# nv-tlabs/ChronoEdit

Hardware: AMD Instinct MI355X
Metric: denoising-steps/sec (higher is better)
Workload: dtype bf16

## Files before the change

### chronoedit_amd/csrc/ce_attn.hip

```cpp
#include <cstdlib>

#include "ce_common.h"

namespace {

constexpr int HD = 128;
constexpr int QW = 32;
constexpr int KVB = 64;
constexpr int K_TILE_BYTES = KVB * HD * 2;
constexpr int VT_TILE_BYTES = HD * KVB * 2;
constexpr int BUF_BYTES = K_TILE_BYTES + VT_TILE_BYTES;
constexpr int OST_ROW = HD * 2 + 16;
constexpr int smem_bytes(int nwave, bool two_seg) {
  const int stage = nwave * QW * OST_ROW;
  return two_seg ? 2 * BUF_BYTES + stage : (stage > 2 * BUF_BYTES ? stage : 2 * BUF_BYTES);
}
constexpr float NEG_BIG = -1.0e30f;

__device__ __forceinline__ int vt_swz(int dv) {
  return ((((dv >> 2) & 7) << 1) | (((dv >> 1) ^ (dv >> 5)) & 1)) ^ (((dv >> 6) & 1) << 1);
}

struct KVSeg {
  const bf16* k;
// ... 1377 lines not shown
#endif
  if (g_attn_nwave == 128 || g_attn_nwave == 129) {
    static bool done4_[CE_MAX_DEVICES] = {};
    bool& done4 = done4_[ce_device_slot()];
    if (!done4) {
      (void)hipFuncSetAttribute((const void*)attn_fwd_w4_kernel, hipFuncAttributeMaxDynamicSharedMemorySize, W4_SMEM);
      done4 = true;
    }
    const int grid4 = (g_attn_nwave == 129 && items > cus) ? (cus & ~7) : items;
    hipLaunchKernelGGL(attn_fwd_w4_kernel, dim3(grid4), dim3(256), W4_SMEM, stream, (const bf16*)Q, (bf16*)O, s0, Nq, H, ldq, ldo, nqb,
                       sl2, batch, blk);
    return (int)hipGetLastError();
  }
  const int grid_vt = items <= 2 * cus ? items : ((2 * cus) & ~7);
  hipLaunchKernelGGL((attn_fwd_sp_kernel<false, true>), dim3(grid_vt), dim3(512), sp_smem_bytes(false), stream, (const bf16*)Q, (bf16*)O,
                     s0, s1, Nq, H, ldq, ldo, nqb, sl2, batch, blk);
  return (int)hipGetLastError();
}

CE_API int ce_attention_vt_bf16(const void* Q, const void* K, const void* Vt, int len, int ldk, int ldvt, void* O, int Nq, int H,
                                    int head_dim, int ldq, int ldo, float softmax_scale, int batch, hipStream_t stream) {
  return attention_vt_launch(Q, K, Vt, len, ldk, ldvt, O, Nq, H, head_dim, ldq, ldo, softmax_scale, batch, 0, 0, 0, stream);
}

CE_API int ce_attention_vt_blocked_bf16(const void* Q, const void* K, const void* Vt, int len, int ldk, int ldvt, void* O, int Nq, int H,
                                            int head_dim, int ldq, int ldo, float softmax_scale, int batch, int blk_rows, int blk_stride,
                                            int vt_sample_cols, hipStream_t stream) {
  if (blk_rows <= 0) return CE_ERR_SHAPE;
  return attention_vt_launch(Q, K, Vt, len, ldk, ldvt, O, Nq, H, head_dim, ldq, ldo, softmax_scale, batch, blk_rows, blk_stride, vt_sample_cols,
                             stream);
}


static int attention_2seg_vt_launch(const void* Q, const void* K1, const void* V1t, int len1, int ldk1, int ldv1t, int vt_cols1,
                                    const void* K2, const void* V2t, int len2, int ldk2, int ldv2t, int vt_cols2, void* O, int Nq,
                                    int H, int head_dim, int ldq, int ldo, float softmax_scale, int batch, void* O8, void* S8, int ldo8,
                                    int q_rows, int k1_rows, int k2_rows, hipStream_t stream, const void* valid1 = nullptr,
                                    const void* w1 = nullptr) {
  if (!Q || !K1 || !V1t || !K2 || !V2t || (!O && !O8)) return CE_ERR_ARG;
  if ((valid1 != nullptr) != (w1 != nullptr) || (valid1 && O8)) return CE_ERR_ARG;
  if ((q_rows != 0 && q_rows < Nq) || (k1_rows != 0 && k1_rows < len1) || (k2_rows != 0 && k2_rows < len2)) return CE_ERR_SHAPE;
  if (k1_rows == 0) vt_cols1 = 0;
  if (k2_rows == 0) vt_cols2 = 0;
  if (head_dim != HD || Nq <= 0 || H <= 0 || len1 <= 0 || len2 <= 0 || batch <= 0 || batch > 65535) return CE_ERR_SHAPE;
  const int c1 = (len1 + KVB - 1) / KVB * KVB, c2 = (len2 + KVB - 1) / KVB * KVB;
  if ((k1_rows != 0 && vt_cols1 < len1) || (k2_rows != 0 && vt_cols2 < len2) || ldv1t < (batch - 1) * vt_cols1 + c1 || ldv2t < (batch - 1) * vt_cols2 + c2)
    return CE_ERR_SHAPE;
  if ((ldq & 7) || (ldo & 7) || (ldk1 & 7) || (ldk2 & 7) || (ldv1t & 7) || (ldv2t & 7) || (vt_cols1 & 1) || (vt_cols2 & 1)) return CE_ERR_ALIGN;
  KVSeg s0{(const bf16*)K1, (const bf16*)V1t, len1, ldk1, ldv1t};
  KVSeg s1{(const bf16*)K2, (const bf16*)V2t, len2, ldk2, ldv2t};
  const float sl2 = softmax_scale * 1.4426950408889634f;
  const int nqb = (Nq + 8 * QW - 1) / (8 * QW);
  static bool done_[CE_MAX_DEVICES] = {};
  bool& done = done_[ce_device_slot()];
  if (!done) {
    (void)hipFuncSetAttribute((const void*)attn_fwd_sp_kernel<true, true>, hipFuncAttributeMaxDynamicSharedMemorySize, sp_smem_bytes(true));
    (void)hipFuncSetAttribute((const void*)attn_fwd_sp_kernel<true, true, true>, hipFuncAttributeMaxDynamicSharedMemorySize, sp_smem_bytes(true));
    (void)hipFuncSetAttribute((const void*)attn_fwd_sp_kernel<true, true, false, true>, hipFuncAttributeMaxDynamicSharedMemorySize, sp_smem_bytes(true));
    done = true;
  }
  const BlkRows blk{0, vt_cols2, 0u, vt_cols1, (unsigned char*)O8, (unsigned char*)S8, ldo8, q_rows, k1_rows, k2_rows,
                    (const int*)valid1, (const float*)w1};
  const int cus = ce_device_cus();
  const int items = nqb * H * batch;
  const int grid = items <= 2 * cus ? items : ((2 * cus) & ~7);
  if (valid1)
    hipLaunchKernelGGL((attn_fwd_sp_kernel<true, true, false, true>), dim3(grid), dim3(512), sp_smem_bytes(true), stream, (const bf16*)Q,
                       (bf16*)O, s0, s1, Nq, H, ldq, ldo, nqb, sl2, batch, blk);
  else if (O8)
    hipLaunchKernelGGL((attn_fwd_sp_kernel<true, true, true>), dim3(grid), dim3(512), sp_smem_bytes(true), stream, (const bf16*)Q,
                       (bf16*)O, s0, s1, Nq, H, ldq, ldo, nqb, sl2, batch, blk);
  else
    hipLaunchKernelGGL((attn_fwd_sp_kernel<true, true>), dim3(grid), dim3(512), sp_smem_bytes(true), stream, (const bf16*)Q, (bf16*)O,
                       s0, s1, Nq, H, ldq, ldo, nqb, sl2, batch, blk);
  return (int)hipGetLastError();
}

CE_API int ce_attention_2seg_vt_bf16(const void* Q, const void* K1, const void* V1t, int len1, int ldk1, int ldv1t, int vt_cols1,
                                         const void* K2, const void* V2t, int len2, int ldk2, int ldv2t, int vt_cols2, void* O, int Nq,
                                         int H, int head_dim, int ldq, int ldo, float softmax_scale, int batch, hipStream_t stream) {
  if (!O) return CE_ERR_ARG;
  return attention_2seg_vt_launch(Q, K1, V1t, len1, ldk1, ldv1t, vt_cols1, K2, V2t, len2, ldk2, ldv2t, vt_cols2, O, Nq, H, head_dim, ldq, ldo,
                                  softmax_scale, batch, nullptr, nullptr, 0, Nq, len1, len2, stream);
}

CE_API int ce_attention_2seg_vt_strided_bf16(const void* Q, const void* K1, const void* V1t, int len1, int ldk1, int ldv1t, int vt_cols1,
                                                 const void* K2, const void* V2t, int len2, int ldk2, int ldv2t, int vt_cols2, void* O, int Nq,
                                                 int H, int head_dim, int ldq, int ldo, float softmax_scale, int batch, int q_rows, int k1_rows,
                                                 int k2_rows, hipStream_t stream) {
  if (!O) return CE_ERR_ARG;
  return attention_2seg_vt_launch(Q, K1, V1t, len1, ldk1, ldv1t, vt_cols1, K2, V2t, len2, ldk2, ldv2t, vt_cols2, O, Nq, H, head_dim, ldq, ldo,
                                  softmax_scale, batch, nullptr, nullptr, 0, q_rows, k1_rows, k2_rows, stream);
}

CE_API int ce_attention_2seg_vt_weighted_bf16(const void* Q, const void* K1, const void* V1t, int len1, int ldk1, int ldv1t, int vt_cols1,
                                                  const void* K2, const void* V2t, int len2, int ldk2, int ldv2t, int vt_cols2, void* O, int Nq,
                                                  int H, int head_dim, int ldq, int ldo, float softmax_scale, int batch, int q_rows, int k1_rows,
                                                  int k2_rows, const void* valid1, const void* w1, hipStream_t stream) {
  if (!O || !valid1 || !w1) return CE_ERR_ARG;
  return attention_2seg_vt_launch(Q, K1, V1t, len1, ldk1, ldv1t, vt_cols1, K2, V2t, len2, ldk2, ldv2t, vt_cols2, O, Nq, H, head_dim, ldq, ldo,
                                  softmax_scale, batch, nullptr, nullptr, 0, q_rows, k1_rows, k2_rows, stream, valid1, w1);
}

CE_API int ce_attention_2seg_vt_quant_bf16(const void* Q, const void* K1, const void* V1t, int len1, int ldk1, int ldv1t, int vt_cols1,
                                               const void* K2, const void* V2t, int len2, int ldk2, int ldv2t, int vt_cols2, void* o8,
                                               void* scale8, int Nq, int H, int head_dim, int ldq, int ldo8, float softmax_scale, int batch,
                                               hipStream_t stream) {
  if (!o8 || !scale8 || (ldo8 & 15) || ((H * head_dim) & 127)) return CE_ERR_ARG;
  return attention_2seg_vt_launch(Q, K1, V1t, len1, ldk1, ldv1t, vt_cols1, K2, V2t, len2, ldk2, ldv2t, vt_cols2, nullptr, Nq, H, head_dim, ldq,
                                  8, softmax_scale, batch, o8, scale8, ldo8, Nq, len1, len2, stream);
}
```

### chronoedit_amd/hiplib.py

```python
from __future__ import annotations

import ctypes
import os
import re
import subprocess
from typing import Dict, List

PKG_DIR = os.path.dirname(os.path.abspath(__file__))
ROOT = os.path.dirname(PKG_DIR)
CSRC = os.path.join(PKG_DIR, "csrc")
LIB_DIR = os.path.join(PKG_DIR, "lib")
LIB_PATH = os.path.join(LIB_DIR, "libchronoedit_hip.so")
DIAG_LIB_PATH = os.path.join(LIB_DIR, "libchronoedit_hip_diag.so")
OBJ_DIR = os.path.join(LIB_DIR, "obj")
HEADER = os.path.join(ROOT, "include", "chronoedit_hip.h")
DIAG_HEADER = os.path.join(ROOT, "include", "chronoedit_hip_diag.h")

DIAG_SOURCES = ["ce_gemm.hip", "ce_gemm256.hip", "ce_attn.hip", "ce_attn_fp8.hip", "ce_gemm_fp8.hip", "ce_gemm_fp8w4.hip"]
DIAG_ONLY_SOURCES = ["ce_attn16.hip"]
SOURCES = ["ce_rowops.hip", "ce_gemm.hip", "ce_gemm256.hip", "ce_gemm256w4.hip", "ce_gemm384.hip", "ce_attn.hip", "ce_attn16.hip", "ce_attn_fp8.hip", "ce_sched.hip", "ce_conv.hip", "ce_enc.hip", "ce_gemm_fp8.hip", "ce_gemm_fp8w4.hip", "ce_comm.hip", "ce_lora.hip", "ce_tea.hip", "ce_image.hip", "ce_region.hip", "ce_sparse.hip", "ce_region_auto.hip", "ce_focus.hip", "ce_autofocus.hip", "ce_preview.hip", "ce_lift.hip", "ce_sketch.hip", "ce_components.hip", "ce_clusters.hip", "ce_layers.hip"]

_c = ctypes
_P, _I, _F = _c.c_void_p, _c.c_int, _c.c_float

SIGNATURES: Dict[str, List] = {
    "ce_ln_affine_bf16": [_P, _P, _P, _P, _I, _I, _I, _I, _F, _I, _I, _P],
    "ce_rmsnorm_rope_bf16": [_P, _P, _P, _P, _P, _I, _I, _I, _I, _F, _I, _P],
    "ce_gemm_bf16": [_P, _P, _P, _P, _I, _P, _P, _I, _I, _I, _I, _I, _I, _I, _I, _I, _c.c_longlong, _I, _c.c_longlong, _P, _c.c_size_t, _P],
    "ce_gemm_bf16_res": [_P, _P, _P, _P, _I, _P, _P, _I, _I, _I, _I, _I, _I, _I, _I, _I, _I, _c.c_longlong, _I, _c.c_longlong, _P, _c.c_size_t, _P],
    "ce_rmsnorm_rope_mxfp8": [_P, _P, _P, _P, _P, _I, _I, _I, _I, _I, _F, _I, _F, _P],
    "ce_v_mxfp8_transpose": [_P, _I, _P, _P, _I, _I, _I, _I, _P],
    "ce_attention_mxfp8": [_P, _P, _P, _P, _P, _P, _P, _I, _I, _I, _I, _I, _I, _I, _I, _I, _P],
    "ce_attention_mxfp8_quant": [_P, _P, _P, _P, _P, _P, _P, _P, _I, _I, _I, _I, _I, _I, _I, _I, _I, _P],
    "ce_attention_mxfp8_add": [_P, _P, _P, _P, _P, _P, _P, _I, _P, _I, _P, _P, _I, _I, _I, _I, _I, _I, _I, _I, _I, _P],
    "ce_rope_scatter_bf16": [_P, _I, _P, _I, _I, _I, _I, _I, _P, _I, _P, _I, _P, _P, _I, _F, _I, _P],
    "ce_patchify_rows_bf16": [_P, _P, _I, _I, _I, _I, _I, _I, _I, _P],
    "ce_comm_load": [ctypes.c_char_p],
    "ce_comm_unique_id": [_P],
    "ce_comm_init": [ctypes.POINTER(ctypes.c_void_p), _P, _I, _I],
    "ce_comm_destroy": [_P],
    "ce_comm_all_to_all": [_P, _P, _P, ctypes.c_size_t, _P],
    "ce_comm_all_gather": [_P, _P, _P, ctypes.c_size_t, _P],
    "ce_ln_affine_fp8": [_P, _P, _P, _P, _P, _I, _I, _I, _I, _F, _I, _I, _P],
    "ce_quant_rows_fp8": [_P, _P, _P, _I, _I, _I, _I, _P],
    "ce_gemm_fp8": [_P, _P, _P, _P, _P, _P, _I, _P, _P, _I, _I, _I, _I, _I, _I, _I, _I, _P, _c.c_size_t, _P],
    "ce_quant_rows_mxfp8": [_P, _P, _P, _I, _I, _I, _I, _P],
    "ce_quant_rows_mxfp8_w": [_P, _P, _P, _I, _I, _I, _I, _P],
    "ce_ln_affine_mxfp8": [_P, _P, _P, _P, _P, _I, _I, _I, _I, _F, _I, _I, _P],
    "ce_gemm_mxfp8": [_P, _P, _P, _P, _P, _P, _I, _P, _P, _I, _I, _I, _I, _I, _I, _I, _I, _P, _c.c_size_t, _P],
    "ce_gemm_mxfp8_gelu_quant": [_P, _P, _P, _P, _P, _P, _P, _I, _I, _I, _I, _I, _I, _P, _c.c_size_t, _P],
    "ce_gemm_batched_bf16": [_P, _P, _P, _P, _I, _I, _I, _I, _I, _I, _I, _I, _I] + [ctypes.c_longlong] * 6 + [_P],
    "ce_im2col_patch2d_bf16": [_P, _P, _I, _I, _I, _I, _I, _I, _P],
    "ce_gather_rows_bf16": [_P, _P, _P, _I, _I, _I, _I, _I, _P],
    "ce_rmsnorm_bf16": [_P, _P, _P, _I, _I, _I, _I, _F, _P],
    "ce_softmax_t5_bf16": [_P, _P, _I, _I, _I, _I, _I, _I, _P, _P, _P, _P],
    "ce_attention_bf16": [_P, _P, _P, _I, _I, _I, _P, _P, _I, _I, _I, _P, _I, _I, _I, _I, _I, _F, _P],
    "ce_attention_batched_bf16": [_P, _P, _P, _I, _I, _I, _P, _P, _I, _I, _I, _P, _I, _I, _I, _I, _I, _F, _I, _P],
    "ce_attention_vt_bf16": [_P, _P, _P, _I, _I, _I, _P, _I, _I, _I, _I, _I, _F, _I, _P],
    "ce_attention_2seg_vt_bf16": [_P, _P, _P, _I, _I, _I, _I, _P, _P, _I, _I, _I, _I, _P, _I, _I, _I, _I, _I, _F, _I, _P],
    "ce_attention_2seg_vt_strided_bf16": [_P, _P, _P, _I, _I, _I, _I, _P, _P, _I, _I, _I, _I, _P, _I, _I, _I, _I, _I, _F, _I, _I, _I, _I, _P],
    "ce_attention_2seg_vt_weighted_bf16": [_P, _P, _P, _I, _I, _I, _I, _P, _P, _I, _I, _I, _I, _P, _I, _I, _I, _I, _I, _F, _I, _I, _I, _I, _P, _P, _P],
    "ce_attention_2seg_vt_quant_bf16": [_P, _P, _P, _I, _I, _I, _I, _P, _P, _I, _I, _I, _I, _P, _P, _I, _I, _I, _I, _I, _F, _I, _P],
    "ce_v_transpose_bf16": [_P, _I, _P, _I, _I, _I, _P],
    "ce_attention_vt_blocked_bf16": [_P, _P, _P, _I, _I, _I, _P, _I, _I, _I, _I, _I, _F, _I, _I, _I, _I, _P],
    "ce_v_transpose_blocked_bf16": [_P, _I, _P, _I, _I, _I, _I, _I, _I, _I, _P],
    "ce_timestep_sinusoid": [_P, _P, _I, _P],
    "ce_timestep_sinusoid_f32": [_P, _P, _I, _P],
    "ce_gemv": [_P, _I, _P, _P, _P, _I, _I, _I, _P],
    "ce_modulation": [_P, _P, _P, _I, _I, _I, _I, _I, _P],
    "ce_patchify_bf16": [_P, _P, _I, _I, _I, _I, _I, _P],
    "ce_unpatchify_bf16": [_P, _P, _I, _I, _I, _I, _I, _P],
    "ce_conv_igemm_bf16": [_P, _I, _P, _P, _P, _I, _P] + [_I] * 16 + [_P],
    "ce_conv3d_head_bf16": [_P, _I, _P, _P, _P, _I] + [_I] * 10 + [_P],
    "ce_gemm_bf16_tile_rows": [_I, _I, _I, _I, _c.c_longlong],
    "ce_zero_border_bf16": [_P, _I, _I, _I, _I, _I, _P],
    "ce_conv3d_gemm_bf16": [_P, _P, _I, _P, _P, _P, _I, _I, _I, _I, _I, _I, _I, _I, _P],
    "ce_conv3d_gemm_rms_silu_bf16": [_P, _P, _I, _P, _P, _P, _P, _I, _I, _I, _I, _I, _I, _I, _P, _I, _P],
    "ce_rms_silu_bf16": [_P, _P, _P, _c.c_longlong, _I, _I, _I, _I, _I, _I, _P],
    "ce_upsample2x_bf16": [_P, _P, _I, _I, _I, _I, _P],
    "ce_softmax_rows_f32_bf16": [_P, _P, _I, _I, _I, _I, _I, _F, _P],
    "ce_attention_1head_bf16": [_P, _P, _P, _P, _I, _I, _I, _I, _I, _I, _I, _F, _P, _c.c_longlong, _P],
    "ce_cfg_unipc_step": [_P, _P, _P, _P, _P, _P, _P, _P, _P, _c.c_longlong, _I, _P],
    "ce_cfg_unipc_step_delta": [_P, _P, _P, _P, _P, _P, _P, _P, _P, _c.c_longlong, _I, _I, _I, _P, _c.c_longlong, _P, _I, _P],
    "ce_lora_merge_bf16": [_P, _I, _P, _I, _I, _I, _I, _P, _P, _P, _P, _P],
    "ce_tea_rel_l1_bf16": [_P, _I, _I, _P, _P],
    "ce_tea_store_bf16": [_P, _P, _c.c_longlong, _P],
    "ce_tea_apply_bf16": [_P, _P, _c.c_longlong, _P],
    "ce_tea_store_dist_bf16": [_P, _P, _P, _P, _P, _c.c_longlong, _c.c_longlong, _P],
    "ce_image_resample_u8": [_P, _P, _I, _I, _I, _I, _P, _P, _I, _P],
    "ce_image_u8_lut_planar": [_P, _I, _I, _I, _I, _I, _I, _P, _P, _I, _P],
    "ce_video_to_u8": [_P, _P, _I, _I, _I, _I, _I, _P],
    "ce_region_weights_u8": [_P, _P, _I, _I, _P],
    "ce_region_blend_f32": [_P, _P, _P, _P, _P, _c.c_longlong, _c.c_longlong, _I, _P],
    "ce_region_composite": [_P, _I, _P, _P, _P, _I, _I, _I, _I, _P],
# ... 152 lines not shown
```

### chronoedit_amd/ops.py

```python
from __future__ import annotations

import ctypes
from typing import Optional

import torch

from . import hiplib

EPI_BIAS, EPI_BIAS_GELU, EPI_GATE_RES, EPI_BIAS_GELU_ERF = 0, 1, 2, 3
EPI_F32, EPI_MUL, EPI_BIAS_ROW, EPI_BIAS_T = 4, 5, 6, 7

_lib = None
_product = None

_KNOB_DEFAULTS = {"ce_set_gemm_variant": -1, "ce_set_attention_waves": 0, "ce_set_gemm_fp8_variant": 1,
                  "ce_set_attention_mxfp8_variant": 1, "ce_set_attention_mxfp8_persistent": 512}
_knobs = dict(_KNOB_DEFAULTS)


def lib():
    global _lib, _product
    if _lib is None:
        _lib = _product = hiplib.load()
        import os
# ... 389 lines not shown


def attention_2seg_vt_shared(q: torch.Tensor, k1: torch.Tensor, v1t: torch.Tensor, len1: int, k2: torch.Tensor, v2t: torch.Tensor, len2: int,
                             heads: int, out: torch.Tensor, batch: int, share_q: bool = False, share1: bool = False, share2: bool = False,
                             cols1: Optional[int] = None, cols2: Optional[int] = None, scale: Optional[float] = None):
    for n, t in (("q", q), ("k1", k1), ("v1t", v1t), ("k2", k2), ("v2t", v2t), ("out", out)):
        _dev(t, torch.bfloat16, n)
    Nq, Dq, ldq = _rows(q, "q")
    _, _, ldk1 = _rows(k1, "k1")
    _, _, ldk2 = _rows(k2, "k2")
    No, Do, ldo = _rows(out, "out")
    nq = Nq if share_q else Nq // batch
    assert Dq == heads * 128 and Do == Dq and v1t.shape[0] == Dq and v2t.shape[0] == Dq and v1t.stride(1) == 1 and v2t.stride(1) == 1
    assert No == batch * nq and (share_q or Nq == batch * nq), (No, Nq, batch)
    assert k1.shape[0] == (1 if share1 else batch) * len1 and k2.shape[0] == (1 if share2 else batch) * len2
    pad = lambda n: (n + 63) // 64 * 64
    if cols1 is None:
        cols1 = 0 if share1 else v1t.shape[1] // batch
    if cols2 is None:
        cols2 = 0 if share2 else v2t.shape[1] // batch
    assert v1t.shape[1] >= (0 if share1 else (batch - 1) * cols1) + pad(len1) and v2t.shape[1] >= (0 if share2 else (batch - 1) * cols2) + pad(len2)
    if scale is None:
        scale = 128 ** -0.5
    st = _prof_begin()
    _check(lib().ce_attention_2seg_vt_strided_bf16(_ptr(q), _ptr(k1), _ptr(v1t), len1, ldk1, v1t.stride(0), int(cols1), _ptr(k2), _ptr(v2t),
                                                   len2, ldk2, v2t.stride(0), int(cols2), _ptr(out), nq, heads, 128, ldq, ldo, float(scale), batch,
                                                   0 if share_q else nq, 0 if share1 else len1, 0 if share2 else len2, _stream()),
           "ce_attention_2seg_vt_strided_bf16")
    tag = ("_sq" if share_q else "") + ("_s1" if share1 else "") + ("_s2" if share2 else "")
    _prof_end(st, f"attention_{nq}x{len1}+{len2}_h{heads}" + (f"_b{batch}" if batch > 1 else "") + tag, 4.0 * nq * (len1 + len2) * 128 * heads * batch)
    return out


def attention_2seg_vt_weighted(q: torch.Tensor, k1: torch.Tensor, v1t: torch.Tensor, len1: int, k2: torch.Tensor, v2t: torch.Tensor, len2: int,
                               heads: int, out: torch.Tensor, batch: int, valid1: torch.Tensor, w1: torch.Tensor, share_q: bool = False,
                               share2: bool = False, cols1: Optional[int] = None, cols2: Optional[int] = None, scale: Optional[float] = None):
    for n, t in (("q", q), ("k1", k1), ("v1t", v1t), ("k2", k2), ("v2t", v2t), ("out", out)):
        _dev(t, torch.bfloat16, n)
    _dev(valid1, torch.int32, "valid1"), _dev(w1, torch.float32, "w1")
    assert valid1.is_contiguous() and w1.is_contiguous() and valid1.numel() == batch and w1.numel() == batch
    Nq, Dq, ldq = _rows(q, "q")
    _, _, ldk1 = _rows(k1, "k1")
    _, _, ldk2 = _rows(k2, "k2")
    No, Do, ldo = _rows(out, "out")
    nq = Nq if share_q else Nq // batch
    assert Dq == heads * 128 and Do == Dq and v1t.shape[0] == Dq and v2t.shape[0] == Dq and v1t.stride(1) == 1 and v2t.stride(1) == 1
    assert No == batch * nq and (share_q or Nq == batch * nq), (No, Nq, batch)
    assert k1.shape[0] == batch * len1 and k2.shape[0] == (1 if share2 else batch) * len2
    pad = lambda n: (n + 63) // 64 * 64
    if cols1 is None:
        cols1 = v1t.shape[1] // batch
    if cols2 is None:
        cols2 = 0 if share2 else v2t.shape[1] // batch
    assert v1t.shape[1] >= (batch - 1) * cols1 + pad(len1) and v2t.shape[1] >= (0 if share2 else (batch - 1) * cols2) + pad(len2)
    if scale is None:
        scale = 128 ** -0.5
    st = _prof_begin()
    _check(lib().ce_attention_2seg_vt_weighted_bf16(_ptr(q), _ptr(k1), _ptr(v1t), len1, ldk1, v1t.stride(0), int(cols1), _ptr(k2), _ptr(v2t),
                                                    len2, ldk2, v2t.stride(0), int(cols2), _ptr(out), nq, heads, 128, ldq, ldo, float(scale), batch,
                                                    0 if share_q else nq, len1, 0 if share2 else len2, _ptr(valid1), _ptr(w1), _stream()),
           "ce_attention_2seg_vt_weighted_bf16")
    tag = ("_sq" if share_q else "") + ("_s2" if share2 else "") + "_w"
    _prof_end(st, f"attention_{nq}x{len1}+{len2}_h{heads}" + (f"_b{batch}" if batch > 1 else "") + tag, 4.0 * nq * (len1 + len2) * 128 * heads * batch)
    return out


def v_transpose_blocked(v: torch.Tensor, heads: int, batch: int, blk_rows: int, n_keys: int, out: Optional[torch.Tensor] = None):
    _dev(v, torch.bfloat16, "v")
    rows, D, ldv = _rows(v, "v")
    assert D == heads * 128 and blk_rows % 64 == 0 and rows % (batch * blk_rows) == 0
    cols = (n_keys + 63) // 64 * 64 + 64
    if out is None:
        out = torch.empty((D, batch * cols), dtype=torch.bfloat16, device=v.device)
    assert out.shape == (D, batch * cols) and out.is_contiguous()
    st = _prof_begin()
    _check(lib().ce_v_transpose_blocked_bf16(_ptr(v), ldv, _ptr(out), out.shape[1], n_keys, heads, batch, blk_rows, batch * blk_rows, cols,
                                             _stream()), "ce_v_transpose_blocked_bf16")
    _prof_end(st, f"v_transpose_{batch * n_keys}x{D}", 4.0 * batch * n_keys * D)
    return out


def attention_vt_blocked(q: torch.Tensor, k: torch.Tensor, vt: torch.Tensor, heads: int, batch: int, blk_rows: int, n_keys: int,
                         out: Optional[torch.Tensor] = None, scale: Optional[float] = None):
    for n, t in (("q", q), ("k", k), ("vt", vt)):
        _dev(t, torch.bfloat16, n)
    rows, Dq, ldq = _rows(q, "q")
    rk, _, ldk = _rows(k, "k")
    assert Dq == heads * 128 and vt.shape[0] == Dq and vt.stride(1) == 1 and rows == rk and rows % (batch * blk_rows) == 0
    nq = rows // batch
    cols = vt.shape[1] // batch
    if out is None:
        out = torch.empty((rows, Dq), dtype=torch.bfloat16, device=q.device)
    _, _, ldo = _rows(out, "out")
    if scale is None:
# ... 1442 lines not shown
```

### include/chronoedit_hip.h

```cpp
#ifndef CHRONOEDIT_HIP_H
#define CHRONOEDIT_HIP_H

#include <stddef.h>
#include <stdint.h>

#ifdef __cplusplus
extern "C" {
#endif

#ifndef __HIP_PLATFORM_AMD__
typedef struct ihipStream_t* hipStream_t;
#endif

#define CE_OK 0
#define CE_ERR_ARG (-1)
#define CE_ERR_SHAPE (-2)
#define CE_ERR_ALIGN (-3)

#define CE_EPI_BIAS 0
#define CE_EPI_BIAS_GELU 1
#define CE_EPI_GATE_RES 2
#define CE_EPI_BIAS_GELU_ERF 3
#define CE_EPI_BIAS_ROW 6
#define CE_EPI_BIAS_T 7
// ... 11 lines not shown

int ce_gemm_bf16_res(const void* A, const void* W, void* C, const float* bias, int epilogue, const float* gate, const void* res,
                     int M, int N, int K, int lda, int ldw, int ldc, int ldres, int gate_rows, int res_rows, int a_seg_k,
                     long long a_seg_stride, int w_seg_k, long long w_seg_stride, void* ws, size_t ws_bytes, hipStream_t stream);



int ce_gemm_bf16_tile_rows(int M, int N, int K, int cus, long long ws_bytes);

int ce_attention_bf16(const void* Q, const void* K1, const void* V1, int len1, int ldk1, int ldv1, const void* K2,
                      const void* V2, int len2, int ldk2, int ldv2, void* O, int Nq, int H, int head_dim, int ldq, int ldo,
                      float softmax_scale, hipStream_t stream);

int ce_attention_batched_bf16(const void* Q, const void* K1, const void* V1, int len1, int ldk1, int ldv1, const void* K2,
                              const void* V2, int len2, int ldk2, int ldv2, void* O, int Nq, int H, int head_dim, int ldq,
                              int ldo, float softmax_scale, int batch, hipStream_t stream);

int ce_attention_vt_bf16(const void* Q, const void* K, const void* Vt, int len, int ldk, int ldvt, void* O, int Nq, int H, int head_dim,
                         int ldq, int ldo, float softmax_scale, int batch, hipStream_t stream);

int ce_attention_2seg_vt_bf16(const void* Q, const void* K1, const void* V1t, int len1, int ldk1, int ldv1t, int vt_cols1, const void* K2,
                              const void* V2t, int len2, int ldk2, int ldv2t, int vt_cols2, void* O, int Nq, int H, int head_dim, int ldq,
                              int ldo, float softmax_scale, int batch, hipStream_t stream);

int ce_attention_2seg_vt_strided_bf16(const void* Q, const void* K1, const void* V1t, int len1, int ldk1, int ldv1t, int vt_cols1,
                                      const void* K2, const void* V2t, int len2, int ldk2, int ldv2t, int vt_cols2, void* O, int Nq, int H,
                                      int head_dim, int ldq, int ldo, float softmax_scale, int batch, int q_rows, int k1_rows, int k2_rows,
                                      hipStream_t stream);

int ce_attention_2seg_vt_weighted_bf16(const void* Q, const void* K1, const void* V1t, int len1, int ldk1, int ldv1t, int vt_cols1,
                                       const void* K2, const void* V2t, int len2, int ldk2, int ldv2t, int vt_cols2, void* O, int Nq, int H,
                                       int head_dim, int ldq, int ldo, float softmax_scale, int batch, int q_rows, int k1_rows, int k2_rows,
                                       const void* valid1, const void* w1, hipStream_t stream);

int ce_attention_2seg_vt_quant_bf16(const void* Q, const void* K1, const void* V1t, int len1, int ldk1, int ldv1t, int vt_cols1, const void* K2,
                                    const void* V2t, int len2, int ldk2, int ldv2t, int vt_cols2, void* o8, void* scale8, int Nq, int H,
                                    int head_dim, int ldq, int ldo8, float softmax_scale, int batch, hipStream_t stream);

int ce_attention_vt_blocked_bf16(const void* Q, const void* K, const void* Vt, int len, int ldk, int ldvt, void* O, int Nq, int H, int head_dim,
                                 int ldq, int ldo, float softmax_scale, int batch, int blk_rows, int blk_stride, int vt_sample_cols,
                                 hipStream_t stream);

int ce_v_transpose_blocked_bf16(const void* v, int ldv, void* vt, int ldvt, int n_keys, int H, int batch, int blk_rows, int blk_stride,
                                int vt_sample_cols, hipStream_t stream);

int ce_v_transpose_bf16(const void* v, int ldv, void* vt, int ldvt, int n_keys, int H, hipStream_t stream);


int ce_timestep_sinusoid(const int64_t* t, float* out, int dim, hipStream_t stream);

int ce_timestep_sinusoid_f32(const float* t, float* out, int dim, hipStream_t stream);

int ce_gemv(const void* W, int w_is_bf16, const float* x, const float* bias, float* y, int N, int K, int flags,
            hipStream_t stream);

int ce_modulation(const float* table, const float* v, float* mod, int L, int J, int D, int v_rows, int one_mask,
                  hipStream_t stream);

int ce_patchify_bf16(const void* x, void* cols, int C, int T, int H, int W, int Kpad, hipStream_t stream);

int ce_patchify_rows_bf16(const void* x, void* cols, int C, int T, int H, int W, int Kpad, int row0, int nrows, hipStream_t stream);

int ce_rope_scatter_bf16(const void* x, int ldx, void* send, int M, int D, int W, int nt, int col0, const float* w0, int col1,
                         const float* w1, int col2, const float* w2, const float* cos_sin, int head_dim, float eps,
                         int rope_rows, hipStream_t stream);

// ... 191 lines not shown
```

Measured before the change: 3.104.

## Add LDS-resident cross-attention kernel for short two-segment weighted attention

Adds a new cross-attention kernel that loads the complete K and V^T of both short key segments (text and image context) into LDS once per block. Each block then loops over many query groups against that resident data instead of streaming KV tiles for every query tile. The existing weighted entry point now calls the dispatcher with form 0 (auto), so the resident path is taken whenever the segment lengths fit in LDS. This cuts repeated global and L2 KV traffic for cross-attention. In exchange it uses up to 160KB of LDS per block, which lowers occupancy, and it adds a fairly complex new kernel with its own masking and weighting logic.

```diff
diff --git a/chronoedit_amd/csrc/ce_attn.hip b/chronoedit_amd/csrc/ce_attn.hip
--- a/chronoedit_amd/csrc/ce_attn.hip
+++ b/chronoedit_amd/csrc/ce_attn.hip
@@ -1433,11 +1433,17 @@
 }
 
 
+extern "C" int ce_attn_cross_resident_fits(int len1, int len2);
+extern "C" int ce_attn_cross_resident_launch(const void* Q, const void* K1, const void* V1t, int len1, int ldk1, int ldv1t, int vt_cols1,
+                                             const void* K2, const void* V2t, int len2, int ldk2, int ldv2t, int vt_cols2, void* O, int Nq,
+                                             int H, int ldq, int ldo, float sl2, int batch, int q_rows, int k1_rows, int k2_rows,
+                                             const void* valid1, const void* w1, int ranges, hipStream_t stream);
+
 static int attention_2seg_vt_launch(const void* Q, const void* K1, const void* V1t, int len1, int ldk1, int ldv1t, int vt_cols1,
                                     const void* K2, const void* V2t, int len2, int ldk2, int ldv2t, int vt_cols2, void* O, int Nq,
                                     int H, int head_dim, int ldq, int ldo, float softmax_scale, int batch, void* O8, void* S8, int ldo8,
                                     int q_rows, int k1_rows, int k2_rows, hipStream_t stream, const void* valid1 = nullptr,
-                                    const void* w1 = nullptr) {
+                                    const void* w1 = nullptr, int form = 1, int ranges = 0, int* path = nullptr) {
   if (!Q || !K1 || !V1t || !K2 || !V2t || (!O && !O8)) return CE_ERR_ARG;
   if ((valid1 != nullptr) != (w1 != nullptr) || (valid1 && O8)) return CE_ERR_ARG;
   if ((q_rows != 0 && q_rows < Nq) || (k1_rows != 0 && k1_rows < len1) || (k2_rows != 0 && k2_rows < len2)) return CE_ERR_SHAPE;
@@ -1451,6 +1457,16 @@
   KVSeg s0{(const bf16*)K1, (const bf16*)V1t, len1, ldk1, ldv1t};
   KVSeg s1{(const bf16*)K2, (const bf16*)V2t, len2, ldk2, ldv2t};
   const float sl2 = softmax_scale * 1.4426950408889634f;
+  if (form < 0 || form > 2 || ranges < 0 || (form != 1 && !valid1)) return CE_ERR_ARG;
+  if (form != 1) {
+    if (ce_attn_cross_resident_fits(len1, len2)) {
+      if (path) *path = 2;
+      return ce_attn_cross_resident_launch(Q, K1, V1t, len1, ldk1, ldv1t, vt_cols1, K2, V2t, len2, ldk2, ldv2t, vt_cols2, O, Nq, H, ldq, ldo, sl2,
+                                           batch, q_rows, k1_rows, k2_rows, valid1, w1, ranges, stream);
+    }
+    if (form == 2) return CE_ERR_SHAPE;
+  }
+  if (path) *path = 1;
   const int nqb = (Nq + 8 * QW - 1) / (8 * QW);
   static bool done_[CE_MAX_DEVICES] = {};
   bool& done = done_[ce_device_slot()];
@@ -1500,7 +1516,17 @@
                                                   int k2_rows, const void* valid1, const void* w1, hipStream_t stream) {
   if (!O || !valid1 || !w1) return CE_ERR_ARG;
   return attention_2seg_vt_launch(Q, K1, V1t, len1, ldk1, ldv1t, vt_cols1, K2, V2t, len2, ldk2, ldv2t, vt_cols2, O, Nq, H, head_dim, ldq, ldo,
-                                  softmax_scale, batch, nullptr, nullptr, 0, q_rows, k1_rows, k2_rows, stream, valid1, w1);
+                                  softmax_scale, batch, nullptr, nullptr, 0, q_rows, k1_rows, k2_rows, stream, valid1, w1, 0);
+}
+
+CE_API int ce_attention_2seg_vt_weighted_select_bf16(const void* Q, const void* K1, const void* V1t, int len1, int ldk1, int ldv1t, int vt_cols1,
+                                                         const void* K2, const void* V2t, int len2, int ldk2, int ldv2t, int vt_cols2, void* O,
+                                                         int Nq, int H, int head_dim, int ldq, int ldo, float softmax_scale, int batch, int q_rows,
+                                                         int k1_rows, int k2_rows, const void* valid1, const void* w1, int form, int ranges,
+                                                         int* path, hipStream_t stream) {
+  if (!O || !valid1 || !w1) return CE_ERR_ARG;
+  return attention_2seg_vt_launch(Q, K1, V1t, len1, ldk1, ldv1t, vt_cols1, K2, V2t, len2, ldk2, ldv2t, vt_cols2, O, Nq, H, head_dim, ldq, ldo,
+                                  softmax_scale, batch, nullptr, nullptr, 0, q_rows, k1_rows, k2_rows, stream, valid1, w1, form, ranges, path);
 }
 
 CE_API int ce_attention_2seg_vt_quant_bf16(const void* Q, const void* K1, const void* V1t, int len1, int ldk1, int ldv1t, int vt_cols1,
diff --git a/chronoedit_amd/csrc/ce_attn_cross.hip b/chronoedit_amd/csrc/ce_attn_cross.hip
--- /dev/null
+++ b/chronoedit_amd/csrc/ce_attn_cross.hip
@@ -0,0 +1,438 @@
+#include <type_traits>
+
+#include "ce_common.h"
+
+namespace {
+
+constexpr int HD = 128;
+constexpr int QW = 32;
+constexpr int KVB = 64;
+constexpr int K_GRP = 1088;
+constexpr int PK_TILE = 16 * K_GRP;
+constexpr int VT_TILE = HD * KVB * 2;
+constexpr int XR_LDS_MAX = 160 * 1024;
+constexpr float NEG_BIG = -1.0e30f;
+constexpr float SP_SPEC_THR = 1024.0f;
+typedef __attribute__((address_space(3))) void lds_void;
+
+__host__ __device__ constexpr int xr_kgroups(int rem) { return rem <= 0 ? 0 : rem <= 4 ? 1 : rem <= 12 ? 3 : rem <= 16 ? 4 : rem <= 32 ? 8 : 16; }
+__host__ __device__ constexpr int xr_k_bytes(int len) { return (len / KVB) * PK_TILE + xr_kgroups(len % KVB) * K_GRP; }
+__host__ __device__ constexpr int xr_v_bytes(int len) { return ((len + KVB - 1) / KVB) * VT_TILE; }
+__host__ __device__ constexpr int xr_lds_bytes(int len1, int len2) {
+  const int text = xr_k_bytes(len1) + xr_v_bytes(len1), iv = xr_v_bytes(len2);
+  return xr_k_bytes(len2) + (text > iv ? text : iv);
+}
+static_assert(PK_TILE - K_GRP <= VT_TILE, "a one-group partial K tile's fragment reads must end inside the V^T tile that follows");
+
+struct XrSeg {
+  const bf16* k;
+  const bf16* v;
+  int len;
+  int ldk;
+  int ldv;
+  int k_rows;
+  int vt_cols;
+};
+struct XrArgs {
+  const bf16* Q;
+  bf16* O;
+  XrSeg seg[2];
+  int Nq, H, ldq, ldo;
+  float scale_log2e;
+  int batch;
+  int q_rows;
+  const int* valid0;
+  const float* w0;
+  int nr;
+  int gpr;
+};
+
+__global__ __launch_bounds__(512) void attn_cross_resident_kernel(XrArgs a) {
+  extern __shared__ __attribute__((aligned(16))) unsigned char smem[];
+  const int tid = threadIdx.x, lane = tid & 63;
+  const int wave = __builtin_amdgcn_readfirstlane(tid >> 6);
+  const int l31 = lane & 31, hh = lane >> 5;
+  const int Nq = a.Nq, ldq = a.ldq, ldo = a.ldo;
+  const float scale_log2e = a.scale_log2e;
+
+  int head, bz, rg;
+  {
+    const int item = blockIdx.x;
+    if ((a.H & 7) == 0) {
+      const int xcd = item & 7, local = item >> 3, hx_n = a.H >> 3;
+      bz = local / (hx_n * a.nr);
+      const int r = local % (hx_n * a.nr);
+      head = xcd + 8 * (r / a.nr);
+      rg = r % a.nr;
+    } else {
+      bz = item / (a.nr * a.H);
+      const int r = item % (a.nr * a.H);
+      head = r / a.nr;
+      rg = r % a.nr;
+    }
+  }
+  const bf16* Q = a.Q + (size_t)bz * a.q_rows * ldq;
+  bf16* O = a.O + (size_t)bz * Nq * ldo;
+  const int hoff = head * HD;
+  const int ngroups = (Nq + QW - 1) / QW;
+  const int g_begin = rg * a.gpr, g_end = min(ngroups, g_begin + a.gpr);
+
+  const XrSeg sg0 = a.seg[0], sg1 = a.seg[1];
+  const int len0 = min(max(a.valid0[bz], 1), sg0.len), len1 = sg1.len;
+  const float w_last0 = a.w0[bz];
+  const int reg_base = xr_k_bytes(len1);
+  const auto k0_rsrc = __builtin_amdgcn_make_buffer_rsrc((void*)(sg0.k + (size_t)bz * sg0.k_rows * sg0.ldk + hoff), 0,
+                                                         (len0 - 1) * sg0.ldk * 2 + HD * 2, 0x00020000);
+  const auto v0_rsrc = __builtin_amdgcn_make_buffer_rsrc((void*)(sg0.v + (size_t)bz * sg0.vt_cols + (size_t)hoff * sg0.ldv), 0,
+                                                         ((HD - 1) * sg0.ldv + (len0 + KVB - 1) / KVB * KVB) * 2, 0x00020000);
+  const auto k1_rsrc = __builtin_amdgcn_make_buffer_rsrc((void*)(sg1.k + (size_t)bz * sg1.k_rows * sg1.ldk + hoff), 0,
+                                                         (len1 - 1) * sg1.ldk * 2 + HD * 2, 0x00020000);
+  const auto v1_rsrc = __builtin_amdgcn_make_buffer_rsrc((void*)(sg1.v + (size_t)bz * sg1.vt_cols + (size_t)hoff * sg1.ldv), 0,
+                                                         ((HD - 1) * sg1.ldv + (len1 + KVB - 1) / KVB * KVB) * 2, 0x00020000);
+  const int kd_row = (lane >> 4) + 4 * ((wave >> 1) & 1) + 8 * (wave & 1) + 16 * (wave >> 2);
+  const int kd_chunk = ((lane & 15) ^ (lane >> 4)) << 4;
+  const int vd_row = 8 * wave + (lane >> 3);
+  const int vd_chunk = ((lane & 7) ^ ((vd_row >> 1) & 7)) << 4;
+  auto dma_k = [&](const __amdgpu_buffer_rsrc_t rs, int ldk, int len, int base) __attribute__((always_inline)) {
+    const int ntiles = (len + KVB - 1) / KVB, nfull = len / KVB, rem = len % KVB;
+    const int voff0 = kd_row * ldk * 2 + kd_chunk, voff1 = voff0 + 32 * ldk * 2;
+    for (int t = 0; t < ntiles; ++t) {
+      const int ng = t < nfull ? 16 : xr_kgroups(rem);
+      if (wave < ng) __builtin_amdgcn_raw_ptr_buffer_load_lds(rs, (lds_void*)(smem + base + t * PK_TILE + wave * K_GRP), 16, voff0, t * KVB * ldk * 2, 0, 0);
+      if (wave + 8 < ng)
+        __builtin_amdgcn_raw_ptr_buffer_load_lds(rs, (lds_void*)(smem + base + t * PK_TILE + (wave + 8) * K_GRP), 16, voff1, t * KVB * ldk * 2, 0, 0);
+    }
+  };
+  auto dma_v = [&](const __amdgpu_buffer_rsrc_t rs, int ldv, int len, int base) __attribute__((always_inline)) {
+    const int ntiles = (len + KVB - 1) / KVB;
+    const int voff0 = vd_row * ldv * 2 + vd_chunk, voff1 = voff0 + 64 * ldv * 2;
+    for (int t = 0; t < ntiles; ++t) {
+      __builtin_amdgcn_raw_ptr_buffer_load_lds(rs, (lds_void*)(smem + base + t * VT_TILE + wave * 1024), 16, voff0, t * (KVB * 2), 0, 0);
+      __builtin_amdgcn_raw_ptr_buffer_load_lds(rs, (lds_void*)(smem + base + t * VT_TILE + (wave + 8) * 1024), 16, voff1, t * (KVB * 2), 0, 0);
+    }
+  };
+
+  const int k_w = l31 & 3;
+  const unsigned char* k_rd = smem + (l31 >> 2) * K_GRP + k_w * 256 + ((hh ^ (k_w & 1)) << 4);
+  const int k_eo[2] = {(k_w >> 1) << 5, ((k_w >> 1) ^ 1) << 5};
+  int vt_off[4];
+#pragma unroll
+  for (int s4 = 0; s4 < 4; ++s4) {
+    const int x = (l31 >> 1) & 7;
+    vt_off[s4] = l31 * 128 + ((2 * (s4 ^ (x >> 1)) + (hh ^ (x & 1))) << 4);
+  }
+
+  auto load_q = [&](bf16x8 (&dst)[8], int g) __attribute__((always_inline)) {
+    const int q0 = g * QW;
+    const bf16* qrow = Q + (size_t)(q0 + l31 < Nq ? q0 + l31 : 0) * ldq + hoff + 8 * hh;
+#pragma unroll
+    for (int ks = 0; ks < 8; ++ks) dst[ks] = *reinterpret_cast<const bf16x8*>(qrow + 16 * ks);
+  };
+
+  dma_k(k1_rsrc, sg1.ldk, len1, 0);
+  bf16x8 qf[8];
+  if (g_begin + wave < g_end) load_q(qf, g_begin + wave);
+
+  for (int c0 = g_begin; c0 < g_end; c0 += 8) {
+    const int g = c0 + wave;
+    const bool active = g < g_end;
+    const int q0 = g * QW;
+    const bool row_ok = active && q0 + l31 < Nq;
+    bf16* orow = O + (size_t)(row_ok ? q0 + l31 : 0) * ldo + hoff + 8 * hh;
+
+    if (c0 != g_begin) {
+      asm volatile("s_waitcnt lgkmcnt(0)" ::: "memory");
+      __builtin_amdgcn_s_barrier();
+    }
+    dma_k(k0_rsrc, sg0.ldk, len0, reg_base);
+    dma_v(v0_rsrc, sg0.ldv, len0, reg_base + xr_k_bytes(len0));
+    asm volatile("s_waitcnt vmcnt(0)" ::: "memory");
+    __builtin_amdgcn_s_barrier();
+
+    if (active) {
+#pragma unroll
+      for (int ks = 0; ks < 8; ++ks) {
+        const u32x4 w = __builtin_bit_cast(u32x4, qf[ks]);
+        u32x4 o;
+#pragma unroll
+        for (int i = 0; i < 4; ++i) o[i] = pack_bf16(bf16lo(w[i]) * scale_log2e, bf16hi(w[i]) * scale_log2e);
+        qf[ks] = __builtin_bit_cast(bf16x8, o);
+      }
+    }
+    u32x4 park[8];
+
+#pragma unroll
+    for (int p = 0; p < 2; ++p) {
+      const int len = p == 0 ? len0 : len1;
+      const float w_last = p == 0 ? w_last0 : 0.f;
+      const int ntiles = (len + KVB - 1) / KVB;
+      const int k_base = p == 0 ? reg_base : 0;
+      const int v_base = p == 0 ? reg_base + xr_k_bytes(len0) : reg_base;
+
+      f32x16 oacc[4];
+#pragma unroll
+      for (int m = 0; m < 4; ++m)
+#pragma unroll
+        for (int r = 0; r < 16; ++r) oacc[m][r] = 0.f;
+      float l_run = 0.f, alpha_prev = 1.0f, mc = 0.f;
+      f32x16 cinit;
+#pragma unroll
+      for (int r = 0; r < 16; ++r) cinit[r] = 0.f;
+      u32x4 ppk[4];
+#pragma unroll
+      for (int s4 = 0; s4 < 4; ++s4) ppk[s4] = u32x4{0u, 0u, 0u, 0u};
+
+      auto tile = [&](const int t, auto first_tile) __attribute__((always_inline)) {
+        constexpr bool FIRST = decltype(first_tile)::value;
+        const unsigned char* kb = k_rd + k_base + t * PK_TILE;
+        const unsigned char* vtb = smem + v_base + (t - 1) * VT_TILE;
+        const f32x16 zero16 = {0.f, 0.f, 0.f, 0.f, 0.f, 0.f, 0.f, 0.f, 0.f, 0.f, 0.f, 0.f, 0.f, 0.f, 0.f, 0.f};
+#define XR_LDK(i) (*reinterpret_cast<const bf16x8*>(kb + k_eo[((i) >> 1) & 1] + ((i) & 1) * 8 * K_GRP + ((i) >> 2) * 64))
+#define XR_LDV(u) (*reinterpret_cast<const bf16x8*>(vtb + vt_off[(u) >> 2] + ((u) & 3) * 4096))
+        f32x16 st[2];
+        if (len - t * KVB <= 32) {
+          constexpr int RING = 4;
+          bf16x8 kf[RING];
+#pragma unroll
+          for (int i = 0; i < RING; ++i) kf[i] = XR_LDK(2 * i);
+#pragma unroll
+          for (int i = 0; i < 8; ++i) {
+            st[0] = __builtin_amdgcn_mfma_f32_32x32x16_bf16(kf[i % RING], qf[i], i == 0 ? cinit : st[0], 0, 0, 0);
+            if (i + RING < 8) kf[i % RING] = XR_LDK(2 * (i + RING));
+            __builtin_amdgcn_sched_barrier(0);
+          }
+#pragma unroll
+          for (int r = 0; r < 16; ++r) st[1][r] = NEG_BIG;
+        } else {
+          constexpr int RING = 4;
+          bf16x8 kf[RING];
+#pragma unroll
+          for (int i = 0; i < RING; ++i) kf[i] = XR_LDK(i);
+#pragma unroll
+          for (int i = 0; i < 16; ++i) {
+            st[i & 1] = __builtin_amdgcn_mfma_f32_32x32x16_bf16(kf[i % RING], qf[i >> 1], i < 2 ? cinit : st[i & 1], 0, 0, 0);
+            if (i + RING < 16) kf[i % RING] = XR_LDK(i + RING);
+            __builtin_amdgcn_sched_barrier(0);
+          }
+        }
+        float alpha = 1.0f;
+        float psum = 0.f;
+        auto mask_tail = [&]() {
+          if ((t + 1) * KVB > len) {
+            int thr = len - t * KVB - 8 * hh;
+            asm volatile("" : "+v"(thr));
+#pragma unroll
+            for (int f = 0; f < 2; ++f)
+#pragma unroll
+              for (int r = 0; r < 16; ++r) {
+                const int c = 32 * f + 16 * (r >> 3) + 4 * ((r >> 2) & 1) + (r & 3);
+                if (c >= thr) st[f][r] = NEG_BIG;
+              }
+          }
+        };
+        auto weigh_last = [&]() {
+          if (p == 0 && t == ntiles - 1 && w_last != 0.f) {
+            int pos = len - 1 - t * KVB - 8 * hh;
+            asm volatile("" : "+v"(pos));
+#pragma unroll
+            for (int f = 0; f < 2; ++f)
+#pragma unroll
+              for (int r = 0; r < 16; ++r) {
+                const int c = 32 * f + 16 * (r >> 3) + 4 * ((r >> 2) & 1) + (r & 3);
+                if (c == pos) st[f][r] += w_last;
+              }
+          }
+        };
+        auto rebase = [&]() {
+          float mx;
+          {
+            float m0 = fmaxf(st[0][0], st[0][1]), m1 = fmaxf(st[0][8], st[0][9]), m2 = fmaxf(st[1][0], st[1][1]), m3 = fmaxf(st[1][8], st[1][9]);
+#pragma unroll
+            for (int r = 2; r < 8; ++r) {
+              m0 = fmaxf(m0, st[0][r]);
+              m1 = fmaxf(m1, st[0][8 + r]);
+              m2 = fmaxf(m2, st[1][r]);
+              m3 = fmaxf(m3, st[1][8 + r]);
+            }
+            mx = fmaxf(fmaxf(m0, m1), fmaxf(m2, m3));
+          }
+          const auto sw = __builtin_amdgcn_permlane32_swap(__float_as_uint(mx), __float_as_uint(mx), false, false);
+          mx = fmaxf(__uint_as_float(sw[0]), __uint_as_float(sw[1]));
+          const float shift = FIRST ? mx : fmaxf(mx, 0.f);
+          alpha = FIRST ? 1.0f : __builtin_amdgcn_exp2f(-shift);
+          mc += shift;
+#pragma unroll
+          for (int f = 0; f < 2; ++f)
+#pragma unroll
+            for (int r = 0; r < 16; ++r) st[f][r] -= shift;
+#pragma unroll
+          for (int r = 0; r < 16; ++r) cinit[r] = -mc;
+        };
+        auto pack_pair = [&](int j) {
+          const f32x2 pr = {st[j >> 3][(2 * j) & 15], st[j >> 3][(2 * j + 1) & 15]};
+          ppk[j >> 2][j & 3] = __builtin_bit_cast(uint32_t, __builtin_convertvector(pr, bf16x2));
+        };
+        mask_tail();
+        weigh_last();
+        if constexpr (FIRST) {
+          rebase();
+#pragma unroll
+          for (int e = 0; e < 32; ++e) st[e >> 4][e & 15] = __builtin_amdgcn_exp2f(st[e >> 4][e & 15]);
+#pragma unroll
+          for (int e = 0; e < 32; ++e) psum += st[e >> 4][e & 15];
+#pragma unroll
+          for (int j = 0; j < 16; ++j) pack_pair(j);
+        } else {
+          if (__any(alpha_prev != 1.0f)) {
+#pragma unroll
+            for (int m = 0; m < 4; ++m)
+#pragma unroll
+              for (int r = 0; r < 16; ++r) oacc[m][r] *= alpha_prev;
+          }
+          {
+            constexpr int VRING = 4;
+            bf16x8 vf[VRING];
+#pragma unroll
+            for (int u = 0; u < VRING; ++u) vf[u] = XR_LDV(u);
+#pragma unroll
+            for (int u = 0; u < 16; ++u) {
+              oacc[u & 3] = __builtin_amdgcn_mfma_f32_32x32x16_bf16(vf[u % VRING], __builtin_bit_cast(bf16x8, ppk[u >> 2]), oacc[u & 3], 0, 0, 0);
+              if (u + VRING < 16) vf[u % VRING] = XR_LDV(u + VRING);
+#pragma unroll
+              for (int e = 2 * u; e < 2 * u + 2; ++e) st[e >> 4][e & 15] = __builtin_amdgcn_exp2f(st[e >> 4][e & 15]);
+              if (u > 0) {
+                psum += st[(u - 1) >> 3][(2 * u - 2) & 15];
+                psum += st[(u - 1) >> 3][(2 * u - 1) & 15];
+              }
+              if (u >= 4) pack_pair(u - 4);
+              __builtin_amdgcn_sched_barrier(0);
+            }
+            psum += st[1][14];
+            psum += st[1][15];
+#pragma unroll
+            for (int j = 12; j < 16; ++j) pack_pair(j);
+          }
+          if (__builtin_expect(__any(psum > SP_SPEC_THR), 0)) {
+#pragma unroll
+            for (int i = 0; i < 16; ++i) {
+              const bf16x8 kfr = XR_LDK(i);
+              st[i & 1] = __builtin_amdgcn_mfma_f32_32x32x16_bf16(kfr, qf[i >> 1], i < 2 ? zero16 : st[i & 1], 0, 0, 0);
+              __builtin_amdgcn_sched_barrier(0);
+            }
+#pragma unroll
+            for (int f = 0; f < 2; ++f)
+#pragma unroll
+              for (int r = 0; r < 16; ++r) st[f][r] -= mc;
+            mask_tail();
+            weigh_last();
+            rebase();
+            psum = 0.f;
+#pragma unroll
+            for (int j = 0; j < 16; ++j) {
+              st[j >> 3][(2 * j) & 15] = __builtin_amdgcn_exp2f(st[j >> 3][(2 * j) & 15]);
+              st[j >> 3][(2 * j + 1) & 15] = __builtin_amdgcn_exp2f(st[j >> 3][(2 * j + 1) & 15]);
+              psum += st[j >> 3][(2 * j) & 15] + st[j >> 3][(2 * j + 1) & 15];
+              pack_pair(j);
+            }
+          }
+        }
+        l_run = l_run * alpha + psum;
+        alpha_prev = alpha;
+#undef XR_LDK
+      };
+
+      if (p == 1) {
+        asm volatile("s_waitcnt lgkmcnt(0)" ::: "memory");
+        __builtin_amdgcn_s_barrier();
+        dma_v(v1_rsrc, sg1.ldv, len1, reg_base);
+      }
+      if (active) tile(0, std::true_type{});
+      if (p == 1) {
+        asm volatile("s_waitcnt vmcnt(0)" ::: "memory");
+        __builtin_amdgcn_s_barrier();
+      }
+      if (active) {
+        for (int t = 1; t < ntiles; ++t) tile(t, std::false_type{});
+        if (__any(alpha_prev != 1.0f)) {
+#pragma unroll
+          for (int m = 0; m < 4; ++m)
+#pragma unroll
+            for (int r = 0; r < 16; ++r) oacc[m][r] *= alpha_prev;
+        }
+        if (p == 1 && g + 8 < g_end) load_q(qf, g + 8);
+        {
+          const unsigned char* vtb = smem + v_base + (ntiles - 1) * VT_TILE;
+          const int nks = (len - (ntiles - 1) * KVB + 15) >> 4;
+#pragma unroll
+          for (int u = 0; u < 16; ++u) {
+            if ((u & 3) == 0 && (u >> 2) >= nks) break;
+            const bf16x8 vfd = XR_LDV(u);
+            oacc[u & 3] = __builtin_amdgcn_mfma_f32_32x32x16_bf16(vfd, __builtin_bit_cast(bf16x8, ppk[u >> 2]), oacc[u & 3], 0, 0, 0);
+            if (u & 1) __builtin_amdgcn_sched_barrier(0);
+          }
+        }
+#undef XR_LDV
+        const float l_tot = l_run + __shfl_xor(l_run, 32, 64);
+        const float inv = 1.0f / l_tot;
+#pragma unroll
+        for (int m = 0; m < 4; ++m)
+#pragma unroll
+          for (int j = 0; j < 2; ++j) {
+            const int a0 = 2 * j, a1 = 2 * j + 1;
+            const uint32_t e0 = pack_bf16(oacc[m][4 * a0 + 0] * inv, oacc[m][4 * a0 + 1] * inv);
+            const uint32_t e1 = pack_bf16(oacc[m][4 * a0 + 2] * inv, oacc[m][4 * a0 + 3] * inv);
+            const uint32_t f0 = pack_bf16(oacc[m][4 * a1 + 0] * inv, oacc[m][4 * a1 + 1] * inv);
+            const uint32_t f1 = pack_bf16(oacc[m][4 * a1 + 2] * inv, oacc[m][4 * a1 + 3] * inv);
+            const auto s0 = __builtin_amdgcn_permlane32_swap(e0, f0, false, false);
+            const auto s1 = __builtin_amdgcn_permlane32_swap(e1, f1, false, false);
+            u32x4 val = {s0[0], s1[0], s0[1], s1[1]};
+            if (p == 0) {
+              park[2 * m + j] = val;
+            } else {
+              const u32x4 pv = park[2 * m + j];
+#pragma unroll
+              for (int i = 0; i < 4; ++i) val[i] = pack_bf16(bf16lo(pv[i]) + bf16lo(val[i]), bf16hi(pv[i]) + bf16hi(val[i]));
+              if (row_ok) *reinterpret_cast<u32x4*>(orow + 32 * m + 16 * j) = val;
+            }
+          }
+      }
+    }
+  }
+}
+
+}
+
+extern "C" int ce_attn_cross_resident_fits(int len1, int len2) { return len1 > 0 && len2 > 0 && xr_lds_bytes(len1, len2) <= XR_LDS_MAX; }
+
+extern "C" int ce_attn_cross_resident_launch(const void* Q, const void* K1, const void* V1t, int len1, int ldk1, int ldv1t, int vt_cols1,
+                                             const void* K2, const void* V2t, int len2, int ldk2, int ldv2t, int vt_cols2, void* O, int Nq,
+                                             int H, int ldq, int ldo, float sl2, int batch, int q_rows, int k1_rows, int k2_rows,
+                                             const void* valid1, const void* w1, int ranges, hipStream_t stream) {
+  if (!ce_attn_cross_resident_fits(len1, len2) || ranges < 0) return CE_ERR_SHAPE;
+  static bool done_[CE_MAX_DEVICES] = {};
+  bool& done = done_[ce_device_slot()];
+  if (!done) {
+    (void)hipFuncSetAttribute((const void*)attn_cross_resident_kernel, hipFuncAttributeMaxDynamicSharedMemorySize, XR_LDS_MAX);
+    done = true;
+  }
+  const int ngroups = (Nq + QW - 1) / QW;
+  int nr = ranges > 0 ? ranges : ce_device_cus() / (batch * H);
+  if (nr < 1) nr = 1;
+  if (nr > ngroups) nr = ngroups;
+  const int gpr = (ngroups + nr - 1) / nr;
+  nr = (ngroups + gpr - 1) / gpr;
+  XrArgs a;
+  a.Q = (const bf16*)Q;
+  a.O = (bf16*)O;
+  a.seg[0] = XrSeg{(const bf16*)K1, (const bf16*)V1t, len1, ldk1, ldv1t, k1_rows, vt_cols1};
+  a.seg[1] = XrSeg{(const bf16*)K2, (const bf16*)V2t, len2, ldk2, ldv2t, k2_rows, vt_cols2};
+  a.Nq = Nq, a.H = H, a.ldq = ldq, a.ldo = ldo;
+  a.scale_log2e = sl2;
+  a.batch = batch;
+  a.q_rows = q_rows;
+  a.valid0 = (const int*)valid1;
+  a.w0 = (const float*)w1;
+  a.nr = nr, a.gpr = gpr;
+  hipLaunchKernelGGL(attn_cross_resident_kernel, dim3(batch * H * nr), dim3(512), xr_lds_bytes(len1, len2), stream, a);
+  return (int)hipGetLastError();
+}
diff --git a/chronoedit_amd/hiplib.py b/chronoedit_amd/hiplib.py
--- a/chronoedit_amd/hiplib.py
+++ b/chronoedit_amd/hiplib.py
@@ -18,7 +18,7 @@
 
 DIAG_SOURCES = ["ce_gemm.hip", "ce_gemm256.hip", "ce_attn.hip", "ce_attn_fp8.hip", "ce_gemm_fp8.hip", "ce_gemm_fp8w4.hip"]
 DIAG_ONLY_SOURCES = ["ce_attn16.hip"]
-SOURCES = ["ce_rowops.hip", "ce_gemm.hip", "ce_gemm256.hip", "ce_gemm256w4.hip", "ce_gemm384.hip", "ce_attn.hip", "ce_attn16.hip", "ce_attn_fp8.hip", "ce_sched.hip", "ce_conv.hip", "ce_enc.hip", "ce_gemm_fp8.hip", "ce_gemm_fp8w4.hip", "ce_comm.hip", "ce_lora.hip", "ce_tea.hip", "ce_image.hip", "ce_region.hip", "ce_sparse.hip", "ce_region_auto.hip", "ce_focus.hip", "ce_autofocus.hip", "ce_preview.hip", "ce_lift.hip", "ce_sketch.hip", "ce_components.hip", "ce_clusters.hip", "ce_layers.hip"]
+SOURCES = ["ce_rowops.hip", "ce_gemm.hip", "ce_gemm256.hip", "ce_gemm256w4.hip", "ce_gemm384.hip", "ce_attn.hip", "ce_attn_cross.hip", "ce_attn16.hip", "ce_attn_fp8.hip", "ce_sched.hip", "ce_conv.hip", "ce_enc.hip", "ce_gemm_fp8.hip", "ce_gemm_fp8w4.hip", "ce_comm.hip", "ce_lora.hip", "ce_tea.hip", "ce_image.hip", "ce_region.hip", "ce_sparse.hip", "ce_region_auto.hip", "ce_focus.hip", "ce_autofocus.hip", "ce_preview.hip", "ce_lift.hip", "ce_sketch.hip", "ce_components.hip", "ce_clusters.hip", "ce_layers.hip"]
 
 _c = ctypes
 _P, _I, _F = _c.c_void_p, _c.c_int, _c.c_float
@@ -60,6 +60,7 @@
     "ce_attention_2seg_vt_bf16": [_P, _P, _P, _I, _I, _I, _I, _P, _P, _I, _I, _I, _I, _P, _I, _I, _I, _I, _I, _F, _I, _P],
     "ce_attention_2seg_vt_strided_bf16": [_P, _P, _P, _I, _I, _I, _I, _P, _P, _I, _I, _I, _I, _P, _I, _I, _I, _I, _I, _F, _I, _I, _I, _I, _P],
     "ce_attention_2seg_vt_weighted_bf16": [_P, _P, _P, _I, _I, _I, _I, _P, _P, _I, _I, _I, _I, _P, _I, _I, _I, _I, _I, _F, _I, _I, _I, _I, _P, _P, _P],
+    "ce_attention_2seg_vt_weighted_select_bf16": [_P, _P, _P, _I, _I, _I, _I, _P, _P, _I, _I, _I, _I, _P, _I, _I, _I, _I, _I, _F, _I, _I, _I, _I, _P, _P, _I, _I, _P, _P],
     "ce_attention_2seg_vt_quant_bf16": [_P, _P, _P, _I, _I, _I, _I, _P, _P, _I, _I, _I, _I, _P, _P, _I, _I, _I, _I, _I, _F, _I, _P],
     "ce_v_transpose_bf16": [_P, _I, _P, _I, _I, _I, _P],
     "ce_attention_vt_blocked_bf16": [_P, _P, _P, _I, _I, _I, _P, _I, _I, _I, _I, _I, _F, _I, _I, _I, _I, _P],
diff --git a/chronoedit_amd/ops.py b/chronoedit_amd/ops.py
--- a/chronoedit_amd/ops.py
+++ b/chronoedit_amd/ops.py
@@ -445,9 +445,14 @@
     return out
 
 
+_CROSS_FORMS = {"auto": 0, "stream": 1, "resident": 2}
+
+
 def attention_2seg_vt_weighted(q: torch.Tensor, k1: torch.Tensor, v1t: torch.Tensor, len1: int, k2: torch.Tensor, v2t: torch.Tensor, len2: int,
                                heads: int, out: torch.Tensor, batch: int, valid1: torch.Tensor, w1: torch.Tensor, share_q: bool = False,
-                               share2: bool = False, cols1: Optional[int] = None, cols2: Optional[int] = None, scale: Optional[float] = None):
+                               share2: bool = False, cols1: Optional[int] = None, cols2: Optional[int] = None, scale: Optional[float] = None,
+                               form: str = "auto", ranges: int = 0, report: Optional[dict] = None):
+    assert form in _CROSS_FORMS and ranges >= 0
     for n, t in (("q", q), ("k1", k1), ("v1t", v1t), ("k2", k2), ("v2t", v2t), ("out", out)):
         _dev(t, torch.bfloat16, n)
     _dev(valid1, torch.int32, "valid1"), _dev(w1, torch.float32, "w1")
@@ -469,10 +474,20 @@
     if scale is None:
         scale = 128 ** -0.5
     st = _prof_begin()
-    _check(lib().ce_attention_2seg_vt_weighted_bf16(_ptr(q), _ptr(k1), _ptr(v1t), len1, ldk1, v1t.stride(0), int(cols1), _ptr(k2), _ptr(v2t),
-                                                    len2, ldk2, v2t.stride(0), int(cols2), _ptr(out), nq, heads, 128, ldq, ldo, float(scale), batch,
-                                                    0 if share_q else nq, len1, 0 if share2 else len2, _ptr(valid1), _ptr(w1), _stream()),
-           "ce_attention_2seg_vt_weighted_bf16")
+    if form == "auto" and ranges == 0 and report is None:
+        _check(lib().ce_attention_2seg_vt_weighted_bf16(_ptr(q), _ptr(k1), _ptr(v1t), len1, ldk1, v1t.stride(0), int(cols1), _ptr(k2), _ptr(v2t),
+                                                        len2, ldk2, v2t.stride(0), int(cols2), _ptr(out), nq, heads, 128, ldq, ldo, float(scale), batch,
+                                                        0 if share_q else nq, len1, 0 if share2 else len2, _ptr(valid1), _ptr(w1), _stream()),
+               "ce_attention_2seg_vt_weighted_bf16")
+    else:
+        path = ctypes.c_int(0)
+        _check(lib().ce_attention_2seg_vt_weighted_select_bf16(_ptr(q), _ptr(k1), _ptr(v1t), len1, ldk1, v1t.stride(0), int(cols1), _ptr(k2),
+                                                               _ptr(v2t), len2, ldk2, v2t.stride(0), int(cols2), _ptr(out), nq, heads, 128, ldq, ldo,
+                                                               float(scale), batch, 0 if share_q else nq, len1, 0 if share2 else len2,
+                                                               _ptr(valid1), _ptr(w1), _CROSS_FORMS[form], int(ranges), ctypes.byref(path),
+                                                               _stream()), "ce_attention_2seg_vt_weighted_select_bf16")
+        if report is not None:
+            report["path"] = {1: "stream", 2: "resident"}[path.value]
     tag = ("_sq" if share_q else "") + ("_s2" if share2 else "") + "_w"
     _prof_end(st, f"attention_{nq}x{len1}+{len2}_h{heads}" + (f"_b{batch}" if batch > 1 else "") + tag, 4.0 * nq * (len1 + len2) * 128 * heads * batch)
     return out
diff --git a/include/chronoedit_hip.h b/include/chronoedit_hip.h
--- a/include/chronoedit_hip.h
+++ b/include/chronoedit_hip.h
@@ -67,6 +67,12 @@
                                        const void* K2, const void* V2t, int len2, int ldk2, int ldv2t, int vt_cols2, void* O, int Nq, int H,
                                        int head_dim, int ldq, int ldo, float softmax_scale, int batch, int q_rows, int k1_rows, int k2_rows,
                                        const void* valid1, const void* w1, hipStream_t stream);
+
+int ce_attention_2seg_vt_weighted_select_bf16(const void* Q, const void* K1, const void* V1t, int len1, int ldk1, int ldv1t, int vt_cols1,
+                                              const void* K2, const void* V2t, int len2, int ldk2, int ldv2t, int vt_cols2, void* O, int Nq,
+                                              int H, int head_dim, int ldq, int ldo, float softmax_scale, int batch, int q_rows, int k1_rows,
+                                              int k2_rows, const void* valid1, const void* w1, int form, int ranges, int* path,
+                                              hipStream_t stream);
 
 int ce_attention_2seg_vt_quant_bf16(const void* Q, const void* K1, const void* V1t, int len1, int ldk1, int ldv1t, int vt_cols1, const void* K2,
                                     const void* V2t, int len2, int ldk2, int ldv2t, int vt_cols2, void* o8, void* scale8, int Nq, int H,
```

Result: no change. 3.119, median of 6 (+0.5%).
